# zhixuan-lin/IODINE

Measured on AMD Instinct MI355X. Metric: refinement_iters_per_s, higher is better.
Workload: dtype f32 tensors; conv products from 3 f16 MFMAs on hi+lo splits: >= 22 bits relative to the 8x16-cell maximum (tile-relative), f32 accumulate; 1 GPU; CLEVR6 128x128, K=7, T=5, batch 32/GPU, train step (forward + backward + fused Adam step, noise drawn inside the step); step=train, global_batch=32, slots=7, iters=5, img_size=128, hip_graph=False

## Files before the change

### include/iodine_hip.h

```cpp
#ifndef IODINE_HIP_H
#define IODINE_HIP_H

#include <stddef.h>

#ifdef __cplusplus
extern "C" {
#endif

#define IODINE_OK 0
#define IODINE_ERR_INVALID 1
#define IODINE_ERR_HIP 2
#define IODINE_ERR_STATE 3
#define IODINE_ERR_WORKSPACE 4

#define IODINE_ABI_VERSION 3

#define IODINE_ENC_POSTERIOR      (1u << 0)
#define IODINE_ENC_GRAD_POST      (1u << 1)
#define IODINE_ENC_IMAGE          (1u << 2)
#define IODINE_ENC_MEANS          (1u << 3)
#define IODINE_ENC_MASK           (1u << 4)
#define IODINE_ENC_MASK_LOGITS    (1u << 5)
#define IODINE_ENC_MASK_POSTERIOR (1u << 6)
#define IODINE_ENC_GRAD_MEANS     (1u << 7)
// ... 200 lines not shown
int iodine_sheet_form(const iodine_sheet_spec* spec, const float* x, const float* pred, const float* mask, const float* mean,
                      const unsigned char* gt, const unsigned char* sheet);
int iodine_render_sheet(void* stream, const iodine_sheet_spec* spec, const float* x, const float* pred, const float* mask,
                        const float* mean, const unsigned char* gt, const unsigned char* slot_color, const unsigned char* gt_color,
                        unsigned char* sheet);

int iodine_set_option(iodine_handle* h, const char* key, double value);
int iodine_profile_read(iodine_handle* h, const char* category, double* total_ms, long long* launches, int reset);
int iodine_debug_copy(iodine_handle* h, void* stream, const char* name, int iter, float* dst, size_t max_floats,
                      size_t* n_floats);

void iodine_linspace_host(int n, float* out);
enum { IODINE_CONV_TILE_F32 = 0, IODINE_CONV_GATHER = 1, IODINE_CONV_TILE_F16 = 2, IODINE_CONV_S2_FWD = 5, IODINE_CONV_S2_DGRAD = 6, IODINE_CONV_WS = 9,
       IODINE_CONV_WS_B = 10 , IODINE_CONV_WINO = 11 , IODINE_CONV_WS_F32 = 12,
       IODINE_CONV_S2_FWD_F32 = 13, IODINE_CONV_S2_DGRAD_F32 = 14, IODINE_CONV_S2WS = 15, IODINE_CONV_S2WS_F32 = 16, IODINE_CONV_WS_1P = 17 };
int iodine_op_conv3x3(void* stream, int mode, const float* in_nhwc, const float* w_oihw, const float* bias,
                      const float* aux, float* out_nhwc, int n, int ih, int iw, int w_o, int w_i, int cin_pad,
                      int cout, int stride, int epi, int transpose_flip);
int iodine_op_dec_out(void* stream, const float* in_nhwc, const float* w_oihw, const float* bias, float* out_nhwc4,
                      int n, int s, int c);
enum { IODINE_DEC_OUT_TILES = 0, IODINE_DEC_OUT_ROWS = 1, IODINE_DEC_OUT_TILES_NOMAX = 2, IODINE_DEC_OUT_ROWS_F32 = 3 };
int iodine_op_dec_out_f16x3(void* stream, const float* in_nhwc, const float* w_oihw, const float* bias, float* out_nhwc4,
                            int n, int s, int c, int variant);
enum { IODINE_WGRAD_STRIDE2_F32 = -2 };
int iodine_op_conv3x3_wgrad(void* stream, const float* in_nhwc, const float* d_nhwc, float* gw_oihw, float* gb, int n,
                            int s, int ci_pad, int ci_real, int co, int stride);

int iodine_op_conv3x3_wgrad_f32(void* stream, const float* in_nhwc, const float* d_nhwc, float* gw_oihw, float* gb, int n,
                                int s, int c);

enum { IODINE_GEN_FWD = 0, IODINE_GEN_DGRAD = 1, IODINE_GEN_WGRAD = 2 };
int iodine_op_gen_conv(void* stream, int mode, const float* in_nhwc, const float* w_oihw, const float* bias, const float* aux,
                       float* out_nhwc, float* gb, int n, int si, int ci, int ldc, int co, int k, int s, int elu);

int iodine_op_gen_conv_tier(int mode, int si, int ci, int ldc, int co, int k, int s);

int iodine_op_gen_l0(void* stream, int mode, const float* z, const float* w_oihw, const float* bias, const float* dpre, float* out,
                     float* gw, float* gb, float* dz, int n, int L, int s, int co, int k, int ld, float alpha);

int iodine_op_gen_conv_f16x3(void* stream, int mode, const float* in_nhwc, const float* w_oihw, const float* bias, const float* aux,
                             float* out_nhwc, float* gb, int n, int si, int ci, int ldc, int co, int k, int s, int elu);

int iodine_op_render_bwd(void* stream, const float* dec_out, const float* g_pred, const float* g_mask, const float* g_mean, float* g_out,
                         int batch, int slots, int pixels, int strict);

int iodine_op_render_bwd_logits(void* stream, const float* dec_out, const float* g_pred, const float* g_mask, const float* g_mean,
                                const float* g_logits, float* g_out, int batch, int slots, int pixels, int strict);
// ... 32 lines not shown
```

### iodine_amd/build.py

```python
from __future__ import annotations

import glob
import os
import subprocess
import sys
from concurrent.futures import ThreadPoolExecutor

HERE = os.path.dirname(os.path.abspath(__file__))
CSRC = os.path.join(HERE, 'csrc')
ROOT = os.path.dirname(HERE)
LIB = os.path.join(HERE, 'libiodine_hip.so')
SOURCES = ['kernels_conv.hip', 'kernels_convws.hip', 'kernels_out.hip', 'kernels_pixel.hip', 'kernels_pixmap.hip', 'kernels_render.hip', 'kernels_misc.hip', 'kernels_clip.hip', 'kernels_objects.hip', 'kernels_chains.hip', 'kernels_sheet.hip', 'kernels_match.hip', 'kernels_batch.hip', 'kernels_edit.hip', 'kernels_predictive.hip', 'kernels_train.hip', 'kernels_wgrad.hip', 'kernels_gemm.hip', 'kernels_headbwd.hip', 'kernels_outbwd.hip', 'kernels_wgradws.hip', 'kernels_wgrad32.hip', 'kernels_refine.hip', 'kernels_refbwd.hip', 'kernels_refws.hip', 'kernels_refl0.hip', 'kernels_pack.hip', 'kernels_generic.hip', 'kernels_gensplit.hip', 'kernels_gens2.hip', 'kernels_genl0.hip', 'iodine_api.cpp', 'iodine_dispatch.cpp', 'iodine_plan.cpp', 'iodine_checks.cpp', 'iodine_params.cpp', 'iodine_train.cpp', 'iodine_pad.cpp', 'iodine_ops.cpp', 'iodine_sheet.cpp']


def _headers():
    return sorted(glob.glob(os.path.join(CSRC, '*.h'))) + [os.path.join(ROOT, 'include', 'iodine_hip.h')]


HEADERS = _headers()
FLAGS = ['--offload-arch=gfx950', '-O3', '-std=c++17', '-fPIC', '-Wall', '-Wno-unused-function',
         '-Wno-unused-result'] + os.environ.get('IODINE_EXTRA_HIPCC_FLAGS', '').split()


def _hipcc() -> str:
    for c in (os.environ.get('HIPCC'), '/opt/rocm/bin/hipcc', 'hipcc'):
        if c and (os.path.isabs(c) and os.path.exists(c) or not os.path.isabs(c)):
            return c
    raise RuntimeError('hipcc not found')


def _stale(target: str, deps) -> bool:
    if not os.path.exists(target):
        return True
    t = os.path.getmtime(target)
    return any(os.path.getmtime(d) > t for d in deps)
# ... 51 lines not shown
```

### iodine_amd/csrc/common.h

```cpp
#pragma once
#include "device.h"
#include "launch.h"
#include <algorithm>
#include <atomic>

inline hipError_t iod_cu_count(int* n_cu)
{
    static std::atomic<int> cache[32];
    int dev = 0;
    hipError_t e = hipGetDevice(&dev);
    if (e != hipSuccess) return e;
    int v = cache[dev & 31].load(std::memory_order_acquire);
    if (!v) {
        e = hipDeviceGetAttribute(&v, hipDeviceAttributeMultiprocessorCount, dev);
        if (e != hipSuccess) return e;
        cache[dev & 31].store(v, std::memory_order_release);
    }
    *n_cu = v;
    return hipSuccess;
}

#ifdef IODINE_XSKIP_HOOK
extern int g_iod_xskip;
#define IOD_XSKIP(bit) do { if (g_iod_xskip & (bit)) return hipSuccess; } while (0)
// ... 252 lines not shown
constexpr int GEN_L0_KMAX = 7;
size_t gen_l0_scratch_floats(int N, int S, int Co, int k);
hipError_t launch_gen_l0_coord(hipStream_t st, const float* wt0, const float* bias, const float* lin, int L, int S, int Co, int k, float* cterm);
hipError_t launch_gen_l0_fwd(hipStream_t st, const float* z, const float* wt0, const float* cterm, float* scratch, float* out, int N, int L, int S,
                             int Co, int k);
hipError_t launch_gen_l0_bwd(hipStream_t st, const float* dpre, const float* z, const float* wt0, const float* lin, float* scratch, int N, int L,
                             int S, int Co, int k, float alpha, float* gw, float* gb, float* dz, int ld);
bool gen_s2_fwd_ok(int k, int Ci, int ldc, int Co);
bool gen_s2_dgrad_ok(int k, int Ci, int ldi, int Co);
bool gen_s2_wgrad_ok(int k, int Ci, int ldc, int Co);
hipError_t launch_gen_s2_fwd(hipStream_t st, const float* in, const float* wt, const float* bias, float* out, int N, int Si, int Ci, int ldc,
                             int Co, int k, int elu, unsigned chmask = 0xffffffffu);
hipError_t launch_gen_s2_dgrad(hipStream_t st, const float* dout, const float* wt, const float* aux, float* din, int N, int Si, int Ci, int ldi,
                               int Co, int k);
hipError_t launch_gen_s2_wgrad(hipStream_t st, const float* in, const float* dout, float* part, int N, int Si, int Ci, int ldc, int Co, int k,
                               int nsl_max, int* nsl_out, unsigned chmask = 0xffffffffu);
hipError_t launch_gen_identity(hipStream_t st, float* m, int rows, int L);
hipError_t launch_ref_unsplit_grad(hipStream_t st, const float* g20, int O, float* gw);
hipError_t launch_enc_join(hipStream_t st, const float* enck, const float* encs, float* enc, int N, int K, int P);
hipError_t launch_conv3x3_s2_dgrad_f16x3(hipStream_t st, const float* d, const void* wpk, const float* wmeta, const float* aux,
                                         float* out, int N, int S, int c, int f32 = 0);
hipError_t launch_conv3x3_s2_wgrad_f16x3(hipStream_t st, const float* a, const float* d, float* part, float* part_b, int N,
                                         int S, int ci_real, int nco, int* nparts, int* cipad, int* nbias_parts,
                                         const float* a2 = nullptr, int kdiv = 0, int f32 = 0);
bool refine_l0_fused_ok(int S, int c, int K);
hipError_t launch_refine_l0_fused(hipStream_t st, const float* x4, const float* dec, const float* lnstat, const float* lin, const void* wk,
                                  const float* wkmeta, const void* ws, const float* wsmeta, const float* bias, float* out, float* enck,
                                  float* encs, int B, int K, int S, int c, float sigma, unsigned chmask, int stable, int joint);
bool conv3x3_s2ws_ok(int S, int c);
hipError_t launch_conv3x3_s2ws_f16x3(hipStream_t st, const float* in, const void* wpk, const float* wmeta, const float* bias, float* out,
                                     int N, int S, int c, int f32 = 0);
bool refine_bwd01_ok(int S, int c);
hipError_t launch_refine_bwd01(hipStream_t st, const float* rd1, const void* wpk, const float* wmeta, const float* act0, const float* enck,
                               const float* encs, float* part, float* part_b, int NT, int S, int c, int kdiv, int* nparts, int* cipad,
                               int* nbias_parts);
hipError_t launch_dec_out_wgrad_gemm_f16x3(hipStream_t st, const float* a, const float* g, float* part, float* part_b, int N,
                                           int S, int c, int* nparts, int* nbias_parts);
hipError_t launch_dec_out_bwd_fused_f16x3(hipStream_t st, const float* a, const float* g, const void* wpk, const float* wmeta,
                                          float* out, float* tmax, float* part, float* part_b, int N, int S, int c,
                                          int* nparts, int* nbias_parts, float alpha = 1.f, int accum = 0);
hipError_t launch_conv3x3_wgrad_f16x3_ws(hipStream_t st, const float* a, const float* d, float* part, float* part_b, int N,
                                         int S, int ci, int nco, int* nparts, int* ncop, int* nbias_parts, float alpha = 1.f, int accum = 0);
```

### iodine_amd/csrc/iodine_api.cpp

```cpp
#include "iodine_internal.h"

extern "C" {

int iodine_abi_version(void) { return IODINE_ABI_VERSION; }

const char* iodine_last_error(const iodine_handle* h) { return h ? h->err.c_str() : g_create_error.c_str(); }

size_t iodine_workspace_bytes(const iodine_handle* h, int batch, int mode)
{
    if (!h || batch < 1) return 0;
    if (h->shim) return pad_workspace_bytes(h, batch, mode);
    Arena q(nullptr); Buffers tmp; plan(h, batch, mode, q, tmp);
    return tmp.bytes;
}

int iodine_set_workspace(iodine_handle* h, void* dev_ptr, size_t bytes)
{
    if (!h) return IODINE_ERR_INVALID;
    if (h->shim) return pad_set_workspace(h, dev_ptr, bytes);
    if (((uintptr_t)dev_ptr & 255) != 0) return h->fail(IODINE_ERR_INVALID, "workspace must be 256-byte aligned");
    h->ws_user = dev_ptr; h->ws_user_bytes = dev_ptr ? bytes : 0;
    h->buf = Buffers();
    h->calls.arena_gone();
    return IODINE_OK;
// ... 106 lines not shown
    if (!strcmp(key, "sigma_grad")) { h->opt.sigma_grad = value != 0; return IODINE_OK; }
    if (!strcmp(key, "input_grad")) {
        if (value != 0 && value != 1 && value != 2 && value != 3) return h->fail(IODINE_ERR_INVALID, "option input_grad: 0, 1 (image), 2 (pixel weights) or 3 (both)");
        h->opt.input_grad = (int)value;
        return IODINE_OK;
    }
    if (!strcmp(key, "stable_encoding")) { h->opt.stable_enc = value != 0; return IODINE_OK; }
    if (!strcmp(key, "joint_likelihood")) {
        if (value != 0 && value != 1) return h->fail(IODINE_ERR_INVALID, "option joint_likelihood: 0 (a mixture per colour channel, the reference) or 1 (one mixture per pixel over RGB)");
        if (h->opt.joint_ll != (int)value && (h->calls.fwd_done || h->calls.diff_kind)) { h->calls.saved_passes_gone(); h->calls.form_changed = true; }
        h->opt.joint_ll = (int)value;
        return IODINE_OK;
    }
    if (!strcmp(key, "refine_split")) { h->opt.refine_split = value != 0; return IODINE_OK; }
    if (!strcmp(key, "head_fused")) { h->opt.head_fused = value != 0; return IODINE_OK; }
    if (!strcmp(key, "refine_bwd_fused")) { h->opt.refine_bwd_fused = value != 0; return IODINE_OK; }
    if (!strcmp(key, "profile_stride")) {
        if (value < 1) return h->fail(IODINE_ERR_INVALID, "profile_stride must be >= 1");
        h->opt.profile_stride = (int)value; return IODINE_OK;
    }
    if (!strcmp(key, "head_mfma")) { h->opt.head_mfma = value != 0; return IODINE_OK; }
    if (!strcmp(key, "refine_l0_fused")) { h->opt.refine_l0_fused = value != 0; return IODINE_OK; }
    if (!strcmp(key, "refine_ws")) { h->opt.refine_ws = value != 0; return IODINE_OK; }
    if (!strcmp(key, "dec_out_rows")) { h->opt.dec_out_rows = value != 0; return IODINE_OK; }
    if (!strcmp(key, "wgrad_accum")) {
        if (h->opt.wgrad_accum != (value != 0)) { h->buf = Buffers(); h->calls.arena_gone(); }
        h->opt.wgrad_accum = value != 0; return IODINE_OK;
    }
    if (!strcmp(key, "conv_variant")) {
        if (value != 1 && value != 6) return h->fail(IODINE_ERR_INVALID, "conv_variant must be 1 (LDS-tiled) or 6 (weight-stationary)");
        if (((int)value == 6) != (h->opt.variant == 6)) h->params_set = false;
        h->opt.variant = (int)value;
        return IODINE_OK;
    }
    if (!strcmp(key, "conv_precision")) {
        if (value != 0 && value != 1 && value != 2)
            return h->fail(IODINE_ERR_INVALID, "conv_precision must be 0 (f32), 1 (f16x3) or 2 (f16x3 with single-product fp16 weight-stationary decoder convs)");
        if (h->opt.precision != (int)value) h->params_set = false;
        h->opt.precision = (int)value;
        return IODINE_OK;
    }
    if (!strcmp(key, "gen_conv_precision")) {
        if (value != 0 && value != 1) return h->fail(IODINE_ERR_INVALID, "gen_conv_precision must be 0 (f32) or 1 (f16x3)");
        if (h->opt.gen_precision != (int)value) h->params_set = false;
        h->opt.gen_precision = (int)value;
        return IODINE_OK;
// ... 511 lines not shown
```

### iodine_amd/csrc/iodine_dispatch.cpp

```cpp
#include "iodine_internal.h"

#ifdef IODINE_XSKIP_HOOK
int g_iod_xskip = 0;
#endif

DecPath dec_path(const iodine_handle* h)
{
    if (h->generic) return DEC_GENERIC;
    const bool ws = h->opt.variant == 6 && h->S >= 16 && (h->S & (h->S - 1)) == 0;
    if (h->opt.precision != 0) return ws ? DEC_WS_F16 : DEC_TILE_F16;
    return ws && (h->Cd == 64 || h->Cd == 32) ? DEC_WS_F32 : DEC_TILE_F32;
}

bool dec_f16(DecPath p) { return p == DEC_WS_F16 || p == DEC_TILE_F16; }
int dec_ws_products(const iodine_handle* h) { return h->opt.precision == 2 ? 1 : 3; }

RefFamily ref_family(const iodine_handle* h)
{
    if (h->gen_ref) return REF_GENERIC;
    for (int l = 0, s = h->S; l < h->Dr; ++l, s /= 2) if (s % 2 != 0) return REF_GATHER;
    return h->opt.precision != 0 ? REF_S2_F16 : REF_S2_F32;
}
bool ref_s2(RefFamily f) { return f == REF_S2_F16 || f == REF_S2_F32; }
bool ref_pack_ws(const iodine_handle* h) { return h->Cr == 64; }
// ... 312 lines not shown
                                                      (float)h->obj.sigma, f.split ? b.encs[i] : nullptr, h->enc_chmask, h->opt.precision == 0, h->opt.stable_enc, h->opt.joint_ll));
    switch (f.fam) {
    case REF_GENERIC:
        PROF(h, st, "gen_conv", launch_gen_conv_fwd(st, in, h->gen.wref[l], h->ref.bias[l], b.ract[i][l], N, s, l == 0 ? 17 : Cr, cip, Cr, h->kr, h->rs, 1,
                                                    l == 0 ? h->enc_chmask : 0xffffffffu));
        break;
    case REF_S2_F16: case REF_S2_F32:
        if (l == 0 && f.split) {
            PROF(h, st, cat, launch_conv3x3_s2_f16x3(st, b.encs[i], h->ref.split_sh.data, h->ref.split_sh.meta, nullptr, b.rmap, B, s, 8, Cr, nullptr, 0, f32));
            PROF(h, st, cat, launch_conv3x3_s2_f16x3(st, b.enck[i], h->ref.split_k.data, h->ref.split_k.meta, h->ref.bias[0], b.ract[i][0], N, s, 12, Cr, b.rmap, h->K, f32));
        } else if (ref_layer_ws(h, f, l, s))
            PROF(h, st, cat, launch_conv3x3_s2ws_f16x3(st, in, h->ref.ws[l].data, h->ref.ws[l].meta, h->ref.bias[l], b.ract[i][l], N, s, Cr, f32));
        else
            PROF(h, st, cat, launch_conv3x3_s2_f16x3(st, in, h->ref.s2_f[l].data, h->ref.s2_f[l].meta, h->ref.bias[l], b.ract[i][l], N, s, cip, Cr, nullptr, 0, f32));
        break;
    case REF_GATHER: PROF(h, st, cat, launch_conv3x3_gather(st, in, h->ref.gather_f[l], h->ref.bias[l], b.ract[i][l], N, s, s, cip, Cr, 2)); break;
    }
    return IODINE_OK;
}

int ref_conv_wgrad(iodine_handle* h, hipStream_t st, int NT, int l, int s, bool split, bool fuse01)
{
    Buffers& b = h->buf;
    const int Cr = h->Cr, cip = l == 0 ? 20 : Cr, ireal = l == 0 ? 17 : Cr, so = ref_out_size(h, s), f32 = h->opt.precision == 0;
    const float* in = l == 0 ? b.enc[0] : b.ract[0][l - 1];
    int nparts = 0, cipad = 0, nb = 0;
    float *gb = h->gacc[h->slot.ref_b[l]], *gw = h->gacc[h->slot.ref_w[l]];
    const bool gather0 = l == 0 && h->n_in < 17;
    float* gw_dst = gather0 ? h->ref.g17 : gw;
    if (gather0) HIPCHK(h, launch_zero_fill(st, h->ref.g17, (size_t)Cr * 17 * h->kr * h->kr));
    switch (ref_family(h)) {
    case REF_GENERIC:
        PROF(h, st, "gen_conv", launch_gen_conv_wgrad(st, in, b.rdpre[l], b.gen_scr, NT, s, ireal, cip, ireal, Cr, h->kr, h->rs, 1.f, gw_dst, gb,
                                                      l == 0 ? h->enc_chmask : 0xffffffffu));
        break;
    case REF_S2_F16: case REF_S2_F32: {
        const bool split0 = l == 0 && split;
        if (split0 && fuse01)
            PROF(h, st, "refine_bwd01", launch_refine_bwd01(st, b.rdpre[1], h->ref.bwd01.data, h->ref.bwd01.meta, b.ract[0][0], b.enck[0], b.encs[0], b.wg_part,
                                                            b.wg_part_b, NT, s, Cr, h->K, &nparts, &cipad, &nb));
        else
            PROF(h, st, "refine_wgrad", launch_conv3x3_s2_wgrad_f16x3(st, split0 ? b.enck[0] : in, b.rdpre[l], b.wg_part, b.wg_part_b, NT, s, cip, Cr, &nparts,
                                                                      &cipad, &nb, split0 ? b.encs[0] : nullptr, split0 ? h->K : 0, f32));
        const int ir = split0 ? 20 : ireal;
        if (split0) HIPCHK(h, launch_zero_fill(st, h->ref.g20, (size_t)Cr * 20 * 9));
        HIPCHK(h, launch_wgrad_reduce(st, b.wg_part, nparts, cipad, Cr, Cr, ir, ir, 1.f, split0 ? h->ref.g20 : gw_dst, b.wg_fold, b.wg_part_b, nb, gb));
        if (split0) HIPCHK(h, launch_ref_unsplit_grad(st, h->ref.g20, Cr, gw_dst));
        break;
    }
    case REF_GATHER:
        PROF(h, st, "refine_wgrad", launch_conv3x3_wgrad_gather(st, in, b.rdpre[l], b.wg_part, NT, s, s, cip, Cr, 2, &nparts, &cipad));
        HIPCHK(h, launch_wgrad_reduce(st, b.wg_part, nparts, cipad, Cr, Cr, ireal, ireal, 1.f, gw_dst, b.wg_fold));
        PROF(h, st, "refine_bias_grad", launch_colsum_tall(st, b.rdpre[l], NT * so * so, Cr, 1.f, gb, b.wg_part_b, (size_t)512 * 64));
        break;
    }
    if (gather0) HIPCHK(h, launch_enc_gather_grad(st, h->ref.g17, Cr, h->n_in, h->enc_map, gw, h->kr * h->kr));
    return IODINE_OK;
}

int ref_conv_dgrad(iodine_handle* h, hipStream_t st, int NT, int l, int s)
{
    Buffers& b = h->buf;
    float *d = b.rdpre[l], *out = b.rdpre[l - 1], *act = b.ract[0][l - 1];
    switch (ref_family(h)) {
    case REF_GENERIC: PROF(h, st, "gen_conv", launch_gen_conv_dgrad(st, d, h->gen.wref[l], act, out, NT, s, h->Cr, h->Cr, h->Cr, h->kr, h->rs)); break;
    case REF_S2_F16: case REF_S2_F32:
// ... 39 lines not shown
```

### iodine_amd/csrc/iodine_internal.h

```cpp
#pragma once
#include "../../include/iodine_hip.h"
#include "common.h"

#include <cmath>
#include <cstdio>
#include <cstring>
#include <list>
#include <string>
#include <vector>

#pragma GCC visibility push(hidden)

extern std::string g_create_error;

struct ParamInfo {
    std::string name;
    int ndim;
    long long dims[4];
    size_t numel() const { size_t n = 1; for (int i = 0; i < ndim; ++i) n *= (size_t)dims[i]; return n; }
};

struct Buffers {
    int B = 0, mode = -1;
    int K = 0, T = 0;
// ... 69 lines not shown
    bool form_changed = false;
    bool redecoded = false;

    void saved_passes_gone() { fwd_done = false; diff_kind = 0; }
    void compute_begins(bool keep_lstm_state = false) { saved_passes_gone(); form_changed = false; redecoded = false; sgrad_n = 0; ig_bits = 0; if (!keep_lstm_state) state_iter = -1; }
    void arena_gone() { saved_passes_gone(); form_changed = false; last_elbo_iter = -1; state_iter = -1; enc_valid = false; redecoded = false; sgrad_n = 0; ig_bits = 0; }
};
#pragma GCC visibility pop

struct Pack { void* data = nullptr; float* meta = nullptr; };

struct Options {
    int precision = 1;
    int variant = 6;
    int gen_precision = 0;
    int out_bwd_fused = 1;
    int fuse_l0 = 1;
    int dec_out_rows = 1;
    int wgrad_accum = 0;
    int refine_split = 1;
    int refine_l0_fused = 1;
    int refine_ws = 1;
    int refine_bwd_fused = 1;
    int head_mfma = 1;
    int head_fused = 1;
    int sigma_grad = 0;
    int input_grad = 0;
    int stable_enc = 0;
    int joint_ll = 0;
    int save_bwd = 0;
    int graph = 0;
    int stop_after = -1;
    int profile = 0;
    int profile_stride = 1;
};


struct DecPacks {
    float *wcls = nullptr, *wclsT = nullptr, *cmap = nullptr;
    std::vector<float*> bias;
    std::vector<Pack> ws_f, ws_b;
    std::vector<Pack> tile_f, tile_b;
    std::vector<float*> tile32_f, tile32_b;
    struct Out {
        float* bias = nullptr;
        Pack gemm, dgrad;
// ... 171 lines not shown
```

### iodine_amd/csrc/iodine_ops.cpp

```cpp
#include "iodine_internal.h"
#include "assign.h"

namespace {
int op_invalid(const char* msg) { g_create_error = msg; return IODINE_ERR_INVALID; }
int launched(const char* who, hipError_t e)
{
    if (e == hipSuccess) return IODINE_OK;
    g_create_error = std::string(who) + ": " + hipGetErrorString(e);
    return IODINE_ERR_HIP;
}
}

extern "C" {

int iodine_adam_step(void* stream, const long long* ptrs_dev, const long long* offsets_dev, int n_tensors, long long total,
                     double lr, double beta1, double beta2, double eps, double weight_decay, int step)
{
    if (!ptrs_dev || !offsets_dev || n_tensors < 1 || total < 1 || step < 1) return op_invalid("iodine_adam_step: bad argument");
    return launched("iodine_adam_step", launch_adam_multi((hipStream_t)stream, ptrs_dev, offsets_dev, n_tensors, total, lr, beta1, beta2, eps,
                                           weight_decay, step));
}

size_t iodine_grad_norm_scratch_bytes(long long total) { return total < 1 ? 0 : grad_norm_scratch_bytes(total); }

// ... 312 lines not shown
    } else if (e == hipSuccess)
        e = variant == IODINE_DEC_OUT_ROWS ? launch_dec_out_rows_f16x3(st, in, p.data, p.meta, bias, out, n, s, c, tin)
                                           : launch_dec_out_stream_f16x3(st, in, p.data, p.meta, bias, out, n, s, c, variant == IODINE_DEC_OUT_TILES_NOMAX ? nullptr : tin);
    return op_done("iodine_op_dec_out_f16x3", st, e);
}

int iodine_op_conv3x3_wgrad(void* stream, const float* in, const float* d, float* gw, float* gb, int n, int s, int ci_pad,
                            int ci_real, int co, int stride)
{
    hipStream_t st = (hipStream_t)stream;
    const int cmax = std::max(std::max(ci_pad, co), 32);
    OpScratch scr("iodine_op_conv3x3_wgrad", {sizeof(float) * 512 * 4 * 9 * cmax * cmax, sizeof(float) * WGRAD_FOLD * 9 * cmax * cmax, sizeof(float) * 512 * 64});
    if (!scr.ok()) return IODINE_ERR_HIP;
    float *part = scr.at(0), *fold = scr.at(1), *part_b = scr.at(2);
    int nparts = 0, cip = 0, nb = 0;
    hipError_t e;
    if (stride == 1 && co == 4) {
        e = launch_dec_out_wgrad_gemm_f16x3(st, in, d, part, part_b, n, s, ci_pad, &nparts, &nb);
        if (e == hipSuccess) e = launch_wgrad_reduce(st, part, nparts, ci_pad, 4, 4, ci_real, ci_real, 1.f, gw, fold);
    } else if (stride == 1) {
        e = launch_conv3x3_wgrad_f16x3_ws(st, in, d, part, part_b, n, s, ci_pad, co, &nparts, &cip, &nb);
        if (e == hipSuccess) e = launch_wgrad_reduce(st, part, nparts, ci_pad, cip, co, ci_real, ci_real, 1.f, gw, fold);
    } else {
        e = launch_conv3x3_s2_wgrad_f16x3(st, in, d, part, part_b, n, s, ci_pad, co, &nparts, &cip, &nb, nullptr, 0, stride == IODINE_WGRAD_STRIDE2_F32);
        if (e == hipSuccess) e = launch_wgrad_reduce(st, part, nparts, cip, co, co, ci_real, ci_real, 1.f, gw, fold);
    }
    if (e == hipSuccess) e = launch_colsum(st, part_b, nb, co, co, 1.f, gb);
    return op_done("iodine_op_conv3x3_wgrad", st, e);
}

int iodine_op_gen_conv(void* stream, int mode, const float* in, const float* w, const float* bias, const float* aux, float* out, float* gb,
                       int n, int si, int ci, int ldc, int co, int k, int s, int elu)
{
    hipStream_t st = (hipStream_t)stream;
    if (mode < IODINE_GEN_FWD || mode > IODINE_GEN_WGRAD || s < 1 || s > 8 || (k != 3 && k != 5 && k != 7) || ldc < ci) return op_invalid("iodine_op_gen_conv: argument");
    const unsigned chmask = (elu & 0x100) ? ((unsigned)elu >> 9) : 0xffffffffu;
    elu &= 1;
    OpScratch scr("iodine_op_gen_conv", {wpk_gen_bytes(k, ldc, co), mode == IODINE_GEN_WGRAD ? gen_wgrad_scratch_floats(ci, co, k) * sizeof(float) : 0});
    if (!scr.ok()) return IODINE_ERR_HIP;
    float* wt = scr.at(0);
    hipError_t e = hipSuccess;
    if (mode == IODINE_GEN_FWD) {
        e = launch_gen_pack_weights(st, w, co, ci, k, wt);
        if (e == hipSuccess) e = launch_gen_conv_fwd(st, in, wt, bias, out, n, si, ci, ldc, co, k, s, elu, chmask);
    } else if (mode == IODINE_GEN_DGRAD) {
        e = launch_gen_pack_weights(st, w, co, ldc, k, wt);
        if (e == hipSuccess) e = launch_gen_conv_dgrad(st, in, wt, aux, out, n, si, ci, ldc, co, k, s);
// ... 258 lines not shown
```

### iodine_amd/csrc/iodine_plan.cpp

```cpp
#include "iodine_internal.h"

void build_param_table(iodine_handle* h)
{
    auto add = [&](const std::string& n, std::initializer_list<long long> d) {
        ParamInfo p; p.name = n; p.ndim = (int)d.size(); int i = 0;
        for (long long v : d) p.dims[i++] = v;
        for (; i < 4; ++i) p.dims[i] = 1;
        h->params.push_back(p);
        return (int)h->params.size() - 1;
    };
    const iodine_config& c = h->cfg;
    ParamSlots& s = h->slot;
    int cin = h->n_in;
    for (int i = 0; i < c.ref_conv_layers; ++i) {
        s.ref_w.push_back(add("refine.mlc.layers." + std::to_string(i) + ".weight", {c.ref_conv_chan, cin, c.ref_kernel_size, c.ref_kernel_size}));
        s.ref_b.push_back(add("refine.mlc.layers." + std::to_string(i) + ".bias", {c.ref_conv_chan}));
        cin = c.ref_conv_chan;
    }
    const long long H = c.ref_mlp_units, L = c.dim_latent;
    s.mlp_w = add("refine.mlp.layers.0.weight", {H, c.ref_conv_chan});
    s.mlp_b = add("refine.mlp.layers.0.bias", {H});
    s.wih = add("refine.lstm.weight_ih", {4 * H, H + 4 * L});
    s.whh = add("refine.lstm.weight_hh", {4 * H, H});
    s.bih = add("refine.lstm.bias_ih", {4 * H});
// ... 189 lines not shown
    h->calls.arena_gone();
    return IODINE_OK;
}

int check_ready(iodine_handle* h, int batch)
{
    if (!h) return IODINE_ERR_INVALID;
    if (!h->params_set) return h->fail(IODINE_ERR_STATE, "iodine_set_params has not been called");
    if (batch < 1) return h->fail(IODINE_ERR_INVALID, "batch must be >= 1");
    const size_t cmax = (size_t)std::max(std::max(h->Cd, h->Cr), 20);
    if ((size_t)batch * h->K * h->P * cmax >= ((size_t)1 << 31))
        return h->fail(IODINE_ERR_INVALID, "batch too large for one device: batch * slots * pixels * channels must stay below 2^31 "
                                           "(shard the images over ranks, iodine_amd.parallel)");
    return IODINE_OK;
}

std::vector<uintptr_t> graph_key(const iodine_handle* h, int entry, int batch, std::initializer_list<const void*> ptrs, const Objective* o,
                                 const PixelWeights* pw)
{
    if (!o) o = &h->obj;
    uint64_t sb, bb;
    memcpy(&sb, &o->sigma, 8); memcpy(&bb, &o->beta, 8);
    std::vector<uintptr_t> k = {(uintptr_t)entry, (uintptr_t)batch, (uintptr_t)h->K, (uintptr_t)h->T, (uintptr_t)h->opt.stop_after, (uintptr_t)h->opt.precision,
                                (uintptr_t)h->opt.variant, (uintptr_t)h->opt.fuse_l0, (uintptr_t)h->opt.out_bwd_fused, (uintptr_t)h->opt.refine_split, (uintptr_t)(h->opt.head_fused | (h->opt.refine_bwd_fused << 1) | (h->opt.refine_ws << 2) | (h->opt.refine_l0_fused << 3) | (h->opt.head_mfma << 4) | (h->opt.wgrad_accum << 5) | (h->opt.dec_out_rows << 6) | (h->opt.gen_precision << 7) | (h->opt.sigma_grad << 8) | (h->opt.stable_enc << 9) | (h->opt.input_grad << 10) | (h->opt.joint_ll << 12)),
                                (uintptr_t)(h->ws_user ? h->ws_user : h->ws_own), (uintptr_t)h->frames};
    k.push_back((uintptr_t)sb); k.push_back((uintptr_t)bb); k.push_back((uintptr_t)o->wgen);
    k.push_back((uintptr_t)(pw ? pw->w : nullptr)); k.push_back((uintptr_t)(pw ? pw->per_frame : 0));
    for (const void* p : ptrs) k.push_back((uintptr_t)p);
    return k;
}
```

### iodine_amd/csrc/kernels_refine.hip

```cpp
#include "common.h"
#include <utility>

namespace {

__host__ __device__ constexpr int s2_ntaps(int sb) { return (1 + (sb >> 1)) * (1 + (sb & 1)); }
__host__ __device__ constexpr int s2_ky(int sb, int j) { return (sb >> 1) ? 2 * (j / (1 + (sb & 1))) : 1; }
__host__ __device__ constexpr int s2_kx(int sb, int j) { return (sb & 1) ? 2 * (j % (1 + (sb & 1))) : 1; }
__host__ __device__ constexpr int s2_off(int mode, int k) { return mode == 0 ? (k == 0 ? 0 : 1) : (k == 0 ? 1 : 0); }
__host__ __device__ constexpr int s2_fwd_sb(int i) { return 3 - i; }

template <int CIN_REAL, int CIN, int COUT, int MODE, int SBT, bool F32>
IOD_DEVINL void conv_s2_body(const float* __restrict__ in, const uint4* __restrict__ wpk, const float* __restrict__ wmeta,
                             const float* __restrict__ bias, const float* __restrict__ aux, float* __restrict__ out,
                             int Sc, int tiles, int kdiv, unsigned char* smem_b, int bid)
{
    constexpr int NC16 = CIN / 16;
    constexpr int NSTAGE = MODE == 0 ? 4 * NC16 : NC16;
    constexpr int NT = COUT / 32;
    constexpr int HALO = 17, NPX = HALO * HALO;
    constexpr int PXS = 80;
    constexpr int IN_BYTES = (NPX + 1) * PXS;
    constexpr int TAP_U4 = 4 * COUT;
    constexpr int NIN = (NPX * 4 + 255) / 256;
    constexpr int NWT = (TAP_U4 + 255) / 256;
// ... 723 lines not shown
                                                                         tiles_y, a2, kdiv);
}

template <int CI_REAL, int CI, int NCO, int TH>
hipError_t launch_s2_wgrad_inst(hipStream_t st, const float* a, const float* d, float* part, float* part_b, int N, int Sc,
                                int* nparts, int* cipad, int* nbias_parts, const float* a2, int kdiv)
{
    constexpr int MT = CI / 32, NTT = NCO / 32, KS = 4 / (MT * NTT);
    constexpr size_t lds = (size_t)(2 * CI * (2 * TH + 1) * 20 + 2 * NCO * (TH * 8 + 4)) * 4 + 32;
    static_assert(lds >= 256 * 16, "bias reduction reuses the planes");
    const int tiles_x = (Sc + 15) / 16, tiles_y = (Sc + TH - 1) / TH, ntiles = N * tiles_x * tiles_y;
    const int blocks = ntiles < 512 ? ntiles : 512;
    *nparts = blocks * KS;
    *cipad = CI;
    *nbias_parts = blocks;
    return iod_launch<conv3x3_s2_wgrad_f16x3_kernel<CI_REAL, CI, NCO, TH>>(st, dim3(blocks), dim3(256), lds, (int)lds, a, d, part, part_b, Sc, ntiles, tiles_x,
                                                                           tiles_y, a2, kdiv);
}

}

hipError_t launch_conv3x3_s2_wgrad_f16x3(hipStream_t st, const float* a, const float* d, float* part, float* part_b, int N,
                                         int S, int ci_real, int nco, int* nparts, int* cipad, int* nbias_parts,
                                         const float* a2, int kdiv, int f32)
{
    IOD_XSKIP(1024);
    if (S % 2 != 0 || S < 2 || (a2 && (ci_real != 20 || kdiv < 1))) return hipErrorInvalidValue;
#define S2W_CASE(CR, CP, CO, TH) \
    if (ci_real == CR && nco == CO) \
        return f32 ? launch_s2_wgrad32_inst<CR, CP, CO, TH>(st, a, d, part, part_b, N, S / 2, nparts, cipad, nbias_parts, a2, kdiv) \
                   : launch_s2_wgrad_inst<CR, CP, CO, TH>(st, a, d, part, part_b, N, S / 2, nparts, cipad, nbias_parts, a2, kdiv);
    S2W_CASE(64, 64, 64, 2) S2W_CASE(20, 32, 64, 4) S2W_CASE(32, 32, 32, 4) S2W_CASE(20, 32, 32, 4)
#undef S2W_CASE
    return hipErrorInvalidValue;
}

namespace {
__device__ __constant__ int c_ref_split_map[20] = {3, 4, 5, 6, 7, 8, 9, 10, 11, 12, 14, -1, 0, 1, 2, 13, 15, 16, -1, -1};

__global__ void ref_split_weights_kernel(const float* __restrict__ w, int O, float* __restrict__ w_slot, float* __restrict__ w_sh)
{
    const int idx = blockIdx.x * blockDim.x + threadIdx.x;
    if (idx >= O * 20 * 9) return;
    const int t = idx % 9, i = (idx / 9) % 20, o = idx / 180;
    const int r = c_ref_split_map[i];
    const float v = r >= 0 ? w[((size_t)o * 17 + r) * 9 + t] : 0.f;
    if (i < 12) w_slot[((size_t)o * 12 + i) * 9 + t] = v;
    else w_sh[((size_t)o * 8 + (i - 12)) * 9 + t] = v;
}

// ... 81 lines not shown
```

Before: 3306 image-refinement-iters/s.

## Add warp-specialized double-buffered pipeline for 64-channel stride-2 refine weight gradient

Adds a new weight-gradient kernel for the 64-to-64 stride-2 refinement conv. Four producer waves prefetch the next tiles into registers, split them into hi/lo f16 and write them into double-buffered LDS. Four consumer waves run the three-MFMA products and carry one persistent accumulator per block, rescaling it when the per-tile scale changes. One block runs per CU, so there are far fewer partial sums to reduce than with the old up-to-512-block split. The aim is to overlap global loads with MFMA work and cut reduction traffic, at the cost of lower occupancy, more registers and extra rescaling arithmetic.

```diff
diff --git a/include/iodine_hip.h b/include/iodine_hip.h
--- a/include/iodine_hip.h
+++ b/include/iodine_hip.h
@@ -246,7 +246,7 @@
 enum { IODINE_DEC_OUT_TILES = 0, IODINE_DEC_OUT_ROWS = 1, IODINE_DEC_OUT_TILES_NOMAX = 2, IODINE_DEC_OUT_ROWS_F32 = 3 };
 int iodine_op_dec_out_f16x3(void* stream, const float* in_nhwc, const float* w_oihw, const float* bias, float* out_nhwc4,
                             int n, int s, int c, int variant);
-enum { IODINE_WGRAD_STRIDE2_F32 = -2 };
+enum { IODINE_WGRAD_STRIDE2_F32 = -2, IODINE_WGRAD_STRIDE2_TILED = -3 };
 int iodine_op_conv3x3_wgrad(void* stream, const float* in_nhwc, const float* d_nhwc, float* gw_oihw, float* gb, int n,
                             int s, int ci_pad, int ci_real, int co, int stride);
 
diff --git a/iodine_amd/build.py b/iodine_amd/build.py
--- a/iodine_amd/build.py
+++ b/iodine_amd/build.py
@@ -10,7 +10,7 @@
 CSRC = os.path.join(HERE, 'csrc')
 ROOT = os.path.dirname(HERE)
 LIB = os.path.join(HERE, 'libiodine_hip.so')
-SOURCES = ['kernels_conv.hip', 'kernels_convws.hip', 'kernels_out.hip', 'kernels_pixel.hip', 'kernels_pixmap.hip', 'kernels_render.hip', 'kernels_misc.hip', 'kernels_clip.hip', 'kernels_objects.hip', 'kernels_chains.hip', 'kernels_sheet.hip', 'kernels_match.hip', 'kernels_batch.hip', 'kernels_edit.hip', 'kernels_predictive.hip', 'kernels_train.hip', 'kernels_wgrad.hip', 'kernels_gemm.hip', 'kernels_headbwd.hip', 'kernels_outbwd.hip', 'kernels_wgradws.hip', 'kernels_wgrad32.hip', 'kernels_refine.hip', 'kernels_refbwd.hip', 'kernels_refws.hip', 'kernels_refl0.hip', 'kernels_pack.hip', 'kernels_generic.hip', 'kernels_gensplit.hip', 'kernels_gens2.hip', 'kernels_genl0.hip', 'iodine_api.cpp', 'iodine_dispatch.cpp', 'iodine_plan.cpp', 'iodine_checks.cpp', 'iodine_params.cpp', 'iodine_train.cpp', 'iodine_pad.cpp', 'iodine_ops.cpp', 'iodine_sheet.cpp']
+SOURCES = ['kernels_conv.hip', 'kernels_convws.hip', 'kernels_out.hip', 'kernels_pixel.hip', 'kernels_pixmap.hip', 'kernels_render.hip', 'kernels_misc.hip', 'kernels_clip.hip', 'kernels_objects.hip', 'kernels_chains.hip', 'kernels_sheet.hip', 'kernels_match.hip', 'kernels_batch.hip', 'kernels_edit.hip', 'kernels_predictive.hip', 'kernels_train.hip', 'kernels_wgrad.hip', 'kernels_gemm.hip', 'kernels_headbwd.hip', 'kernels_outbwd.hip', 'kernels_wgradws.hip', 'kernels_wgrad32.hip', 'kernels_refine.hip', 'kernels_refwgrad.hip', 'kernels_refbwd.hip', 'kernels_refws.hip', 'kernels_refl0.hip', 'kernels_pack.hip', 'kernels_generic.hip', 'kernels_gensplit.hip', 'kernels_gens2.hip', 'kernels_genl0.hip', 'iodine_api.cpp', 'iodine_dispatch.cpp', 'iodine_plan.cpp', 'iodine_checks.cpp', 'iodine_params.cpp', 'iodine_train.cpp', 'iodine_pad.cpp', 'iodine_ops.cpp', 'iodine_sheet.cpp']
 
 
 def _headers():
diff --git a/iodine_amd/csrc/common.h b/iodine_amd/csrc/common.h
--- a/iodine_amd/csrc/common.h
+++ b/iodine_amd/csrc/common.h
@@ -298,7 +298,10 @@
                                          float* out, int N, int S, int c, int f32 = 0);
 hipError_t launch_conv3x3_s2_wgrad_f16x3(hipStream_t st, const float* a, const float* d, float* part, float* part_b, int N,
                                          int S, int ci_real, int nco, int* nparts, int* cipad, int* nbias_parts,
-                                         const float* a2 = nullptr, int kdiv = 0, int f32 = 0);
+                                         const float* a2 = nullptr, int kdiv = 0, int form = 0);
+enum { S2_WGRAD_TILED = 0, S2_WGRAD_F32 = 1, S2_WGRAD_PIPE = 2 };
+hipError_t launch_s2_wgrad_pipe64(hipStream_t st, const float* a, const float* d, float* part, float* part_b, int N, int Sc, int* nparts,
+                                  int* cipad, int* nbias_parts);
 bool refine_l0_fused_ok(int S, int c, int K);
 hipError_t launch_refine_l0_fused(hipStream_t st, const float* x4, const float* dec, const float* lnstat, const float* lin, const void* wk,
                                   const float* wkmeta, const void* ws, const float* wsmeta, const float* bias, float* out, float* enck,
diff --git a/iodine_amd/csrc/iodine_api.cpp b/iodine_amd/csrc/iodine_api.cpp
--- a/iodine_amd/csrc/iodine_api.cpp
+++ b/iodine_amd/csrc/iodine_api.cpp
@@ -152,6 +152,7 @@
     if (!strcmp(key, "head_mfma")) { h->opt.head_mfma = value != 0; return IODINE_OK; }
     if (!strcmp(key, "refine_l0_fused")) { h->opt.refine_l0_fused = value != 0; return IODINE_OK; }
     if (!strcmp(key, "refine_ws")) { h->opt.refine_ws = value != 0; return IODINE_OK; }
+    if (!strcmp(key, "refine_wgrad_pipe")) { h->opt.refine_wgrad_pipe = value != 0; return IODINE_OK; }
     if (!strcmp(key, "dec_out_rows")) { h->opt.dec_out_rows = value != 0; return IODINE_OK; }
     if (!strcmp(key, "wgrad_accum")) {
         if (h->opt.wgrad_accum != (value != 0)) { h->buf = Buffers(); h->calls.arena_gone(); }
diff --git a/iodine_amd/csrc/iodine_dispatch.cpp b/iodine_amd/csrc/iodine_dispatch.cpp
--- a/iodine_amd/csrc/iodine_dispatch.cpp
+++ b/iodine_amd/csrc/iodine_dispatch.cpp
@@ -358,7 +358,8 @@
 int ref_conv_wgrad(iodine_handle* h, hipStream_t st, int NT, int l, int s, bool split, bool fuse01)
 {
     Buffers& b = h->buf;
-    const int Cr = h->Cr, cip = l == 0 ? 20 : Cr, ireal = l == 0 ? 17 : Cr, so = ref_out_size(h, s), f32 = h->opt.precision == 0;
+    const int Cr = h->Cr, cip = l == 0 ? 20 : Cr, ireal = l == 0 ? 17 : Cr, so = ref_out_size(h, s);
+    const int form = h->opt.precision == 0 ? S2_WGRAD_F32 : h->opt.refine_wgrad_pipe ? S2_WGRAD_PIPE : S2_WGRAD_TILED;
     const float* in = l == 0 ? b.enc[0] : b.ract[0][l - 1];
     int nparts = 0, cipad = 0, nb = 0;
     float *gb = h->gacc[h->slot.ref_b[l]], *gw = h->gacc[h->slot.ref_w[l]];
@@ -377,7 +378,7 @@
                                                             b.wg_part_b, NT, s, Cr, h->K, &nparts, &cipad, &nb));
         else
             PROF(h, st, "refine_wgrad", launch_conv3x3_s2_wgrad_f16x3(st, split0 ? b.enck[0] : in, b.rdpre[l], b.wg_part, b.wg_part_b, NT, s, cip, Cr, &nparts,
-                                                                      &cipad, &nb, split0 ? b.encs[0] : nullptr, split0 ? h->K : 0, f32));
+                                                                      &cipad, &nb, split0 ? b.encs[0] : nullptr, split0 ? h->K : 0, form));
         const int ir = split0 ? 20 : ireal;
         if (split0) HIPCHK(h, launch_zero_fill(st, h->ref.g20, (size_t)Cr * 20 * 9));
         HIPCHK(h, launch_wgrad_reduce(st, b.wg_part, nparts, cipad, Cr, Cr, ir, ir, 1.f, split0 ? h->ref.g20 : gw_dst, b.wg_fold, b.wg_part_b, nb, gb));
diff --git a/iodine_amd/csrc/iodine_internal.h b/iodine_amd/csrc/iodine_internal.h
--- a/iodine_amd/csrc/iodine_internal.h
+++ b/iodine_amd/csrc/iodine_internal.h
@@ -115,6 +115,7 @@
     int refine_l0_fused = 1;
     int refine_ws = 1;
     int refine_bwd_fused = 1;
+    int refine_wgrad_pipe = 1;
     int head_mfma = 1;
     int head_fused = 1;
     int sigma_grad = 0;
diff --git a/iodine_amd/csrc/iodine_ops.cpp b/iodine_amd/csrc/iodine_ops.cpp
--- a/iodine_amd/csrc/iodine_ops.cpp
+++ b/iodine_amd/csrc/iodine_ops.cpp
@@ -358,7 +358,8 @@
         e = launch_conv3x3_wgrad_f16x3_ws(st, in, d, part, part_b, n, s, ci_pad, co, &nparts, &cip, &nb);
         if (e == hipSuccess) e = launch_wgrad_reduce(st, part, nparts, ci_pad, cip, co, ci_real, ci_real, 1.f, gw, fold);
     } else {
-        e = launch_conv3x3_s2_wgrad_f16x3(st, in, d, part, part_b, n, s, ci_pad, co, &nparts, &cip, &nb, nullptr, 0, stride == IODINE_WGRAD_STRIDE2_F32);
+        e = launch_conv3x3_s2_wgrad_f16x3(st, in, d, part, part_b, n, s, ci_pad, co, &nparts, &cip, &nb, nullptr, 0,
+                                          stride == IODINE_WGRAD_STRIDE2_F32 ? S2_WGRAD_F32 : stride == IODINE_WGRAD_STRIDE2_TILED ? S2_WGRAD_TILED : S2_WGRAD_PIPE);
         if (e == hipSuccess) e = launch_wgrad_reduce(st, part, nparts, cip, co, co, ci_real, ci_real, 1.f, gw, fold);
     }
     if (e == hipSuccess) e = launch_colsum(st, part_b, nb, co, co, 1.f, gb);
diff --git a/iodine_amd/csrc/iodine_plan.cpp b/iodine_amd/csrc/iodine_plan.cpp
--- a/iodine_amd/csrc/iodine_plan.cpp
+++ b/iodine_amd/csrc/iodine_plan.cpp
@@ -235,7 +235,7 @@
     uint64_t sb, bb;
     memcpy(&sb, &o->sigma, 8); memcpy(&bb, &o->beta, 8);
     std::vector<uintptr_t> k = {(uintptr_t)entry, (uintptr_t)batch, (uintptr_t)h->K, (uintptr_t)h->T, (uintptr_t)h->opt.stop_after, (uintptr_t)h->opt.precision,
-                                (uintptr_t)h->opt.variant, (uintptr_t)h->opt.fuse_l0, (uintptr_t)h->opt.out_bwd_fused, (uintptr_t)h->opt.refine_split, (uintptr_t)(h->opt.head_fused | (h->opt.refine_bwd_fused << 1) | (h->opt.refine_ws << 2) | (h->opt.refine_l0_fused << 3) | (h->opt.head_mfma << 4) | (h->opt.wgrad_accum << 5) | (h->opt.dec_out_rows << 6) | (h->opt.gen_precision << 7) | (h->opt.sigma_grad << 8) | (h->opt.stable_enc << 9) | (h->opt.input_grad << 10) | (h->opt.joint_ll << 12)),
+                                (uintptr_t)h->opt.variant, (uintptr_t)h->opt.fuse_l0, (uintptr_t)h->opt.out_bwd_fused, (uintptr_t)h->opt.refine_split, (uintptr_t)(h->opt.head_fused | (h->opt.refine_bwd_fused << 1) | (h->opt.refine_ws << 2) | (h->opt.refine_l0_fused << 3) | (h->opt.head_mfma << 4) | (h->opt.wgrad_accum << 5) | (h->opt.dec_out_rows << 6) | (h->opt.gen_precision << 7) | (h->opt.sigma_grad << 8) | (h->opt.stable_enc << 9) | (h->opt.input_grad << 10) | (h->opt.joint_ll << 12) | (h->opt.refine_wgrad_pipe << 13)),
                                 (uintptr_t)(h->ws_user ? h->ws_user : h->ws_own), (uintptr_t)h->frames};
     k.push_back((uintptr_t)sb); k.push_back((uintptr_t)bb); k.push_back((uintptr_t)o->wgen);
     k.push_back((uintptr_t)(pw ? pw->w : nullptr)); k.push_back((uintptr_t)(pw ? pw->per_frame : 0));
diff --git a/iodine_amd/csrc/kernels_refine.hip b/iodine_amd/csrc/kernels_refine.hip
--- a/iodine_amd/csrc/kernels_refine.hip
+++ b/iodine_amd/csrc/kernels_refine.hip
@@ -769,10 +769,12 @@
 
 hipError_t launch_conv3x3_s2_wgrad_f16x3(hipStream_t st, const float* a, const float* d, float* part, float* part_b, int N,
                                          int S, int ci_real, int nco, int* nparts, int* cipad, int* nbias_parts,
-                                         const float* a2, int kdiv, int f32)
+                                         const float* a2, int kdiv, int form)
 {
     IOD_XSKIP(1024);
     if (S % 2 != 0 || S < 2 || (a2 && (ci_real != 20 || kdiv < 1))) return hipErrorInvalidValue;
+    const bool f32 = form == S2_WGRAD_F32;
+    if (form == S2_WGRAD_PIPE && ci_real == 64 && nco == 64 && S <= 2048) return launch_s2_wgrad_pipe64(st, a, d, part, part_b, N, S / 2, nparts, cipad, nbias_parts);
 #define S2W_CASE(CR, CP, CO, TH) \
     if (ci_real == CR && nco == CO) \
         return f32 ? launch_s2_wgrad32_inst<CR, CP, CO, TH>(st, a, d, part, part_b, N, S / 2, nparts, cipad, nbias_parts, a2, kdiv) \
diff --git a/iodine_amd/csrc/kernels_refwgrad.hip b/iodine_amd/csrc/kernels_refwgrad.hip
--- /dev/null
+++ b/iodine_amd/csrc/kernels_refwgrad.hip
@@ -0,0 +1,234 @@
+#include "common.h"
+#include <algorithm>
+
+namespace {
+
+constexpr int WP_C = 64, WP_TH = 2, WP_HR = 2 * WP_TH + 1, WP_NTHR = 512, WP_NPROD = 256;
+constexpr int WP_APL = WP_HR * 20, WP_DPL = WP_TH * 8 + 4;
+constexpr int WP_BUF = 2 * WP_C * WP_APL + 2 * WP_C * WP_DPL;
+constexpr size_t WP_LDS = (size_t)2 * WP_BUF * 4 + 2 * 8 * 4;
+static_assert((WP_APL / 4) % 2 == 1 && (WP_DPL / 4) % 2 == 1, "plane strides");
+static_assert(WP_BUF * 4 >= WP_NPROD * 16, "bias reduction reuses a buffer");
+
+__global__ __launch_bounds__(WP_NTHR, 1)
+void conv3x3_s2_wgrad_f16x3_kernel_pipe(const float* __restrict__ a, const float* __restrict__ d, float* __restrict__ part,
+                                        float* __restrict__ part_b, int Sc, int ntiles, int tiles_x, int tiles_y)
+{
+    constexpr int C = WP_C, TH = WP_TH, HR = WP_HR, APL = WP_APL, DPL = WP_DPL;
+    constexpr int C4 = C / 4;
+    constexpr int NA_UNITS = HR * 17 * C4, ND_UNITS = TH * 8 * C4;
+    constexpr int NAU = (NA_UNITS + WP_NPROD - 1) / WP_NPROD;
+    static_assert(ND_UNITS == WP_NPROD, "one gradient unit per producer thread");
+
+    extern __shared__ __attribute__((aligned(16))) unsigned smem_wp[];
+    float* s_max = reinterpret_cast<float*>(smem_wp + 2 * WP_BUF);
+
+    const int tid = threadIdx.x;
+    const int lane = tid & 63, wv = tid >> 6;
+    const int Sf = 2 * Sc;
+    const int t0 = (int)((long long)ntiles * blockIdx.x / gridDim.x), t1 = (int)((long long)ntiles * (blockIdx.x + 1) / gridDim.x);
+    const int L = t1 - t0, LB = (L + 1) & ~1;
+    float4 bsum = make_float4(0.f, 0.f, 0.f, 0.f);
+    float sa = 1.f, sd = 1.f;
+    auto next_scales = [&](int nb) {
+        const float* mx = s_max + nb * 8;
+        sa = tile_scale(fmaxf(fmaxf(mx[0], mx[1]), fmaxf(mx[2], mx[3])), sa);
+        sd = tile_scale(fmaxf(fmaxf(mx[4], mx[5]), fmaxf(mx[6], mx[7])), sd);
+    };
+
+    if (wv < 4) {
+        const int c4 = tid % C4;
+        int a_row[NAU], a_cx[NAU];
+#pragma unroll
+        for (int k = 0; k < NAU; ++k) {
+            const int u = tid + k * WP_NPROD, tt = u / C4, slot = tt % 17;
+            a_row[k] = u < NA_UNITS ? tt / 17 : 1 << 20;
+            a_cx[k] = slot == 0 ? -3 : (slot <= 8 ? 4 * (slot - 1) + 1 : 4 * (slot - 9));
+        }
+        const int d_p = (tid / C4) % 8, d_row = tid / C4 / 8;
+        const int rot = (c4 >> 1) & 3;
+
+        constexpr unsigned OOR = 0x80000000u;
+        auto bload = [](__amdgpu_buffer_rsrc_t r, unsigned off) {
+            const u32x4 v = __builtin_amdgcn_raw_buffer_load_b128(r, (int)off, 0, 0);
+            return make_float4(__uint_as_float(v.x), __uint_as_float(v.y), __uint_as_float(v.z), __uint_as_float(v.w));
+        };
+        int ty = t0 % tiles_y, tx = (t0 / tiles_y) % tiles_x, n = t0 / tiles_y / tiles_x;
+        auto load_tile = [&](float4 (&ra)[NAU][2], float4 (&rd)[2], bool live) {
+            const __amdgpu_buffer_rsrc_t rs_a = __builtin_amdgcn_make_buffer_rsrc(const_cast<float*>(a + (live ? (size_t)n * Sf * Sf * C : 0)), 0, live ? Sf * Sf * C * 4 : 0, 0x00020000);
+            const __amdgpu_buffer_rsrc_t rs_d = __builtin_amdgcn_make_buffer_rsrc(const_cast<float*>(d + (live ? (size_t)n * Sc * Sc * C : 0)), 0, live ? Sc * Sc * C * 4 : 0, 0x00020000);
+            const int fy0 = 2 * ty * TH - 1, fxb = 32 * tx;
+#pragma unroll
+            for (int k = 0; k < NAU; ++k) {
+                const int fy = fy0 + a_row[k], fx0 = fxb + a_cx[k], fx1 = fx0 + 2;
+                const unsigned rowoff = (unsigned)fy * (unsigned)Sf * (C * 4) + c4 * 16;
+                const bool rok = (unsigned)fy < (unsigned)Sf;
+                ra[k][0] = bload(rs_a, rok && (unsigned)fx0 < (unsigned)Sf ? rowoff + (unsigned)fx0 * (C * 4) : OOR);
+                ra[k][1] = bload(rs_a, rok && (unsigned)fx1 < (unsigned)Sf ? rowoff + (unsigned)fx1 * (C * 4) : OOR);
+            }
+            {
+                const int gy = ty * TH + d_row, gx = tx * 16 + 2 * d_p;
+                const unsigned rowoff = (unsigned)gy * (unsigned)Sc * (C * 4) + c4 * 16;
+                const bool rok = (unsigned)gy < (unsigned)Sc;
+                rd[0] = bload(rs_d, rok && gx < Sc ? rowoff + (unsigned)gx * (C * 4) : OOR);
+                rd[1] = bload(rs_d, rok && gx + 1 < Sc ? rowoff + (unsigned)(gx + 1) * (C * 4) : OOR);
+            }
+            if (++ty == tiles_y) { ty = 0; if (++tx == tiles_x) { tx = 0; ++n; } }
+        };
+        auto produce = [&](float4 (&ra)[NAU][2], float4 (&rd)[2], int j, int nb) {
+            float ma = 0.f, md = 0.f;
+#pragma unroll
+            for (int k = 0; k < NAU; ++k)
+#pragma unroll
+                for (int q = 0; q < 2; ++q)
+                    ma = fmaxf(ma, fmaxf(fmaxf(fabsf(ra[k][q].x), fabsf(ra[k][q].y)), fmaxf(fabsf(ra[k][q].z), fabsf(ra[k][q].w))));
+#pragma unroll
+            for (int q = 0; q < 2; ++q) {
+                md = fmaxf(md, fmaxf(fmaxf(fabsf(rd[q].x), fabsf(rd[q].y)), fmaxf(fabsf(rd[q].z), fabsf(rd[q].w))));
+                bsum.x += rd[q].x; bsum.y += rd[q].y; bsum.z += rd[q].z; bsum.w += rd[q].w;
+            }
+            ma = wave_max_f32(ma);
+            md = wave_max_f32(md);
+            if (lane == 0) { s_max[nb * 8 + wv] = ma; s_max[nb * 8 + 4 + wv] = md; }
+            __syncthreads();
+            next_scales(nb);
+            unsigned* s_a = smem_wp + nb * WP_BUF;
+            unsigned* s_d = s_a + 2 * C * APL;
+#pragma unroll
+            for (int k = 0; k < NAU; ++k) {
+                const int u = tid + k * WP_NPROD;
+                if (u < NA_UNITS && j < L) {
+                    const int tt = u / C4, slot = tt % 17, row = tt / 17;
+                    const float4 q0 = rot4(ra[k][0], rot), q1 = rot4(ra[k][1], rot);
+                    const float x0[4] = {q0.x, q0.y, q0.z, q0.w}, x1[4] = {q1.x, q1.y, q1.z, q1.w};
+#pragma unroll
+                    for (int e = 0; e < 4; ++e) {
+                        unsigned lo;
+                        const unsigned hi = pack_hi_lo(x0[e] * sa, x1[e] * sa, lo);
+                        const int ch = c4 * 4 + ((e + rot) & 3);
+                        s_a[(0 * C + ch) * APL + row * 20 + slot + 3] = hi;
+                        s_a[(1 * C + ch) * APL + row * 20 + slot + 3] = lo;
+                    }
+                }
+            }
+            if (j < L) {
+                const float4 q0 = rot4(rd[0], rot), q1 = rot4(rd[1], rot);
+                const float x0[4] = {q0.x, q0.y, q0.z, q0.w}, x1[4] = {q1.x, q1.y, q1.z, q1.w};
+#pragma unroll
+                for (int e = 0; e < 4; ++e) {
+                    unsigned lo;
+                    const unsigned hi = pack_hi_lo(x0[e] * sd, x1[e] * sd, lo);
+                    const int ch = c4 * 4 + ((e + rot) & 3);
+                    s_d[(0 * C + ch) * DPL + d_row * 8 + d_p] = hi;
+                    s_d[(1 * C + ch) * DPL + d_row * 8 + d_p] = lo;
+                }
+            }
+            load_tile(ra, rd, j + 2 < L);
+        };
+        float4 ra0[NAU][2], rd0[2], ra1[NAU][2], rd1[2];
+        load_tile(ra0, rd0, 0 < L);
+        load_tile(ra1, rd1, 1 < L);
+        for (int j = 0; j < LB; j += 2) {
+            produce(ra0, rd0, j, 0);
+            produce(ra1, rd1, j + 1, 1);
+        }
+        __syncthreads();
+    } else {
+        const int kh = lane >> 5, li = lane & 31;
+        const int mi = wv & 1, ni = (wv >> 1) & 1;
+        const int ci = mi * 32 + li, co = ni * 32 + li;
+        f32x16 acc[9];
+#pragma unroll
+        for (int t = 0; t < 9; ++t)
+#pragma unroll
+            for (int r = 0; r < 16; ++r) acc[t][r] = 0.f;
+        float acc_prod = 1.f;
+        for (int j = 0; j <= LB; ++j) {
+            __syncthreads();
+            float prod = acc_prod;
+            if (j < L) { next_scales(j & 1); prod = sa * sd; }
+            if (j >= 1 && j <= L) {
+                const unsigned* s_a = smem_wp + ((j - 1) & 1) * WP_BUF;
+                const unsigned* s_d = s_a + 2 * C * APL;
+#pragma unroll
+                for (int r = 0; r < TH; ++r) {
+                    f16x8 bh, bl;
+                    {
+                        const uint4 vb_h = *reinterpret_cast<const uint4*>(s_d + (0 * C + co) * DPL + r * 8 + 4 * kh);
+                        const uint4 vb_l = *reinterpret_cast<const uint4*>(s_d + (1 * C + co) * DPL + r * 8 + 4 * kh);
+                        __builtin_memcpy(&bh, &vb_h, 16); __builtin_memcpy(&bl, &vb_l, 16);
+                    }
+#pragma unroll
+                    for (int ky = 0; ky < 3; ++ky) {
+                        f16x8 A[2][3];
+#pragma unroll
+                        for (int term = 0; term < 2; ++term) {
+                            const unsigned* pl = s_a + (term * C + ci) * APL + (2 * r + ky) * 20;
+                            const uint4 vo = *reinterpret_cast<const uint4*>(pl + 4 + 4 * kh);
+                            const uint4 ve = *reinterpret_cast<const uint4*>(pl + 12 + 4 * kh);
+                            const unsigned prev = pl[3 + 4 * kh] & 0xffff0000u;
+                            uint4 m1;
+                            m1.x = __builtin_amdgcn_alignbit(vo.x, prev, 16);
+                            m1.y = __builtin_amdgcn_alignbit(vo.y, vo.x, 16);
+                            m1.z = __builtin_amdgcn_alignbit(vo.z, vo.y, 16);
+                            m1.w = __builtin_amdgcn_alignbit(vo.w, vo.z, 16);
+                            __builtin_memcpy(&A[term][0], &m1, 16);
+                            __builtin_memcpy(&A[term][1], &ve, 16);
+                            __builtin_memcpy(&A[term][2], &vo, 16);
+                        }
+#pragma unroll
+                        for (int kx = 0; kx < 3; ++kx) {
+                            const int tap = ky * 3 + kx;
+                            acc[tap] = __builtin_amdgcn_mfma_f32_32x32x16_f16(A[1][kx], bh, acc[tap], 0, 0, 0);
+                            acc[tap] = __builtin_amdgcn_mfma_f32_32x32x16_f16(A[0][kx], bl, acc[tap], 0, 0, 0);
+                            acc[tap] = __builtin_amdgcn_mfma_f32_32x32x16_f16(A[0][kx], bh, acc[tap], 0, 0, 0);
+                        }
+                    }
+                }
+            }
+            if (prod != acc_prod) {
+                const float r = prod / acc_prod;
+#pragma unroll
+                for (int tp = 0; tp < 9; ++tp)
+#pragma unroll
+                    for (int q = 0; q < 16; ++q) acc[tp][q] *= r;
+                acc_prod = prod;
+            }
+        }
+        const float inv = 1.f / acc_prod;
+        float* pw = part + (size_t)blockIdx.x * 9 * C * C;
+#pragma unroll
+        for (int tap = 0; tap < 9; ++tap)
+#pragma unroll
+            for (int r = 0; r < 16; ++r) {
+                const int cr = mi * 32 + (r & 3) + 8 * (r >> 2) + 4 * kh;
+                pw[((size_t)tap * C + cr) * C + ni * 32 + li] = acc[tap][r] * inv;
+            }
+    }
+
+    __syncthreads();
+    float4* s_red = reinterpret_cast<float4*>(smem_wp);
+    if (tid < WP_NPROD) s_red[tid] = bsum;
+    __syncthreads();
+    if (tid < C4) {
+        float4 t4 = make_float4(0.f, 0.f, 0.f, 0.f);
+        for (int j = tid; j < WP_NPROD; j += C4) { const float4 v = s_red[j]; t4.x += v.x; t4.y += v.y; t4.z += v.z; t4.w += v.w; }
+        *reinterpret_cast<float4*>(part_b + (size_t)blockIdx.x * C + tid * 4) = t4;
+    }
+}
+
+}
+
+hipError_t launch_s2_wgrad_pipe64(hipStream_t st, const float* a, const float* d, float* part, float* part_b, int N, int Sc, int* nparts,
+                                  int* cipad, int* nbias_parts)
+{
+    int n_cu = 0;
+    if (hipError_t e = iod_cu_count(&n_cu); e != hipSuccess) return e;
+    const int tiles_x = (Sc + 15) / 16, tiles_y = (Sc + WP_TH - 1) / WP_TH, ntiles = N * tiles_x * tiles_y;
+    const int blocks = std::max(1, std::min(ntiles, std::min(n_cu, 512)));
+    *nparts = blocks;
+    *cipad = WP_C;
+    *nbias_parts = blocks;
+    return iod_launch<conv3x3_s2_wgrad_f16x3_kernel_pipe>(st, dim3(blocks), dim3(WP_NTHR), WP_LDS, (int)WP_LDS, a, d, part, part_b, Sc, ntiles, tiles_x,
+                                                          tiles_y);
+}
```

Result: no change. 3318 image-refinement-iters/s, median of 6 (+0.3%).
